# G-Research/ahocorasick_rs

Measured on NVIDIA H100. Metric: haystack_GB_per_s_scanned_find_matches_as_indexes, higher is better.
Workload: dtype u8

## Files before the change

### ahocorasick_rs_b200/csrc/capi.cu

```cuda
#include <atomic>
#include <cstdio>
#include <cstdlib>
#include <cstring>
#include <stdexcept>
#include <string>
#include <utility>
#include <vector>

#include <cooperative_groups.h>

#include "repair.cuh"
#include "scan_staged.cuh"
#include "scan_global.cuh"
#include "scan_sieve.cuh"
#include "tokens.cuh"

namespace acb {

template <int MODE, bool CP>
__global__ void __launch_bounds__(128) scan_plain_kernel(DevImage im, Batch B, Sink out) {
    for (int64_t h = (int64_t)blockIdx.x * blockDim.x + threadIdx.x; h < B.n_haystacks; h += (int64_t)gridDim.x * blockDim.x) {
        const int64_t hs = B.offsets[h], he = B.offsets[h + 1];
        PieceCtx c;
        c.base = B.bytes + hs;
// ... 46 lines not shown
    for (int d = 1; d < 32; d <<= 1) {
        unsigned long long y = __shfl_up_sync(0xffffffffu, x, d);
        if (lane >= d) x += y;
    }
    if (lane == 31) warp_sums[warp] = x;
    __syncthreads();
    if (warp == 0) {
        unsigned long long w = lane < kScanThreads / 32 ? warp_sums[lane] : 0;
#pragma unroll
        for (int d = 1; d < kScanThreads / 32; d <<= 1) {
            unsigned long long y = __shfl_up_sync(0xffffffffu, w, d);
            if (lane >= d) w += y;
        }
        if (lane < kScanThreads / 32) warp_sums[lane] = w;
    }
    __syncthreads();
    const unsigned long long before = warp ? warp_sums[warp - 1] : 0;
    *total = warp_sums[kScanThreads / 32 - 1];
    __syncthreads();
    return before + x - v;
}

template <bool PAIR>
__device__ __forceinline__ unsigned long long scan_item(const uint32_t *in, uint32_t stride, uint64_t i) {
    if (PAIR) {
        const uint2 v = *reinterpret_cast<const uint2 *>(in + i * stride);
        return (unsigned long long)v.x + v.y;
    }
    return in[i * stride];
}

template <bool PAIR>
__device__ __forceinline__ void tile_sum_body(const uint32_t *in, uint32_t stride, uint64_t n, unsigned long long *tile_sums, uint64_t tile,
                                              uint32_t *dense) {
    const uint64_t base = tile * kScanTile + (uint64_t)threadIdx.x * kScanItems;
    unsigned long long v = 0;
#pragma unroll
    for (int i = 0; i < kScanItems; i++)
        if (base + i < n) {
            const unsigned long long x = scan_item<PAIR>(in, stride, base + i);
            if (dense) dense[base + i] = (uint32_t)x;
            v += x;
        }
    unsigned long long total;
    block_exclusive_scan(v, &total);
    if (threadIdx.x == 0) tile_sums[tile] = total;
}

__device__ __forceinline__ unsigned long long tile_prefix(const unsigned long long *tile_sums, uint64_t tile) {
    unsigned long long v = 0;
    for (uint64_t i = threadIdx.x; i < tile; i += kScanThreads) v += tile_sums[i];
    unsigned long long total;
    block_exclusive_scan(v, &total);
    return total;
}

template <bool PAIR>
__device__ __forceinline__ void tile_apply_body(const uint32_t *in, uint32_t stride, uint64_t n, const unsigned long long *tile_sums,
                                                unsigned long long *out, uint64_t tile) {
    const unsigned long long tile_start = tile_prefix(tile_sums, tile);
    const uint64_t base = tile * kScanTile + (uint64_t)threadIdx.x * kScanItems;
    unsigned long long vals[kScanItems], v = 0;
#pragma unroll
    for (int i = 0; i < kScanItems; i++) {
        vals[i] = base + i < n ? scan_item<PAIR>(in, stride, base + i) : 0;
        v += vals[i];
    }
    unsigned long long total;
    unsigned long long run = tile_start + block_exclusive_scan(v, &total);
#pragma unroll
    for (int i = 0; i < kScanItems; i++) {
        if (base + i < n) out[base + i] = run;
        run += vals[i];
        if (base + i + 1 == n) out[n] = run;
    }
}

constexpr int kAccQueue = 0;
constexpr int kAccContFar = 1;
constexpr int kAccRaw = 2;
constexpr int kAccGroups = 3;
constexpr int kAccTraps = 4;
constexpr int kAccRepairs = 5;
constexpr int kAccWords = 8;
constexpr int kAnyScratchWords = 3;

constexpr unsigned kPathFarCp = 1u;
constexpr unsigned kPathSearch = 2u;
constexpr unsigned kPathRepaired = 4u;

struct EpilogueArgs {
    DevImage im;
    Batch B;
    SegPlan P;
    Sink out;
    SegOut seg;
    const uint32_t *counts;
    uint64_t n_items;
    uint8_t *masks;
    unsigned long long *tile_sums, *unit_offsets;
    unsigned long long *cont_tiles, *cont_cum;
    unsigned long long *totals, *acc;
    const acb_match *raw;
    const uint32_t *raw_seq, *raw_unit, *raw_aux;
    unsigned long long raw_cap;
    const uint32_t *pat_cplen;
    acb_match *out_buf;
    unsigned long long out_cap;
    unsigned long long *match_offsets;
    unsigned int *need_repair;
    int do_repair;
};

__device__ __forceinline__ void count_tile(const EpilogueArgs &E, uint64_t tile, bool check, bool with_c0, unsigned int &dirty) {
    const uint64_t n = E.n_items;
    const uint64_t base = tile * kScanTile + (uint64_t)threadIdx.x * kScanItems;
    uint32_t x[kScanItems];
    if (base + kScanItems <= n && !with_c0) {
        const uint4 a = *reinterpret_cast<const uint4 *>(E.counts + base), b = *reinterpret_cast<const uint4 *>(E.counts + base + 4);
        x[0] = a.x, x[1] = a.y, x[2] = a.z, x[3] = a.w, x[4] = b.x, x[5] = b.y, x[6] = b.z, x[7] = b.w;
    } else {
#pragma unroll
        for (int i = 0; i < kScanItems; i++) x[i] = base + i < n ? E.counts[base + i] + (with_c0 ? E.seg.count0[base + i] : 0u) : 0u;
    }
    unsigned long long v = 0;
    uint32_t bits = 0;
#pragma unroll
    for (int i = 0; i < kScanItems; i++) {
        v += x[i];
        bits |= (x[i] != 0u) << i;
    }
    if (check && base < n) {
        uint32_t prev_end = base ? E.seg.key[base - 1].y : kNoState;
#pragma unroll
        for (int i = 0; i < kScanItems; i++)
            if (base + i < n) {
                const uint2 k = E.seg.key[base + i];
                dirty |= (base + i > 0 && k.x != kNoState && k.x != prev_end) ? 1u : 0u;
                prev_end = k.y;
            }
    }
    if (base < n) E.masks[base / kScanItems] = (uint8_t)bits;
    unsigned long long total;
    block_exclusive_scan(v, &total);
    if (threadIdx.x == 0) E.tile_sums[tile] = total;
}

__device__ __forceinline__ void offsets_tile(const EpilogueArgs &E, uint64_t tile, bool with_c0) {
    const uint64_t n = E.n_items;
    const unsigned long long tile_start = tile_prefix(E.tile_sums, tile);
    const uint64_t base = tile * kScanTile + (uint64_t)threadIdx.x * kScanItems;
    const uint32_t bits = base < n ? E.masks[base / kScanItems] : 0u;
    uint32_t x[kScanItems];
    unsigned long long v = 0;
#pragma unroll
    for (int i = 0; i < kScanItems; i++) {
        x[i] = (bits >> i) & 1u ? E.counts[base + i] + (with_c0 ? E.seg.count0[base + i] : 0u) : 0u;
        v += x[i];
    }
    unsigned long long total;
    unsigned long long run = tile_start + block_exclusive_scan(v, &total);
#pragma unroll
    for (int i = 0; i < kScanItems; i++) {
        if ((bits >> i) & 1u) E.unit_offsets[base + i] = run;
        run += x[i];
        if (base + i + 1 == n) E.unit_offsets[n] = run;
    }
}

__device__ __forceinline__ void order_body(const EpilogueArgs &E, unsigned long long raw_total, bool codepoints, bool repaired, bool far) {
    const bool segments = E.seg.key != nullptr;
    const unsigned long long n = raw_total < E.raw_cap ? raw_total : E.raw_cap;
    for (unsigned long long i = (unsigned long long)blockIdx.x * blockDim.x + threadIdx.x; i < n;
         i += (unsigned long long)gridDim.x * blockDim.x) {
        const uint32_t u = E.raw_unit[i];
        uint32_t seq = E.raw_seq[i];
        unsigned long long dst;
        if (segments) {
            const uint32_t k = u >> 1;
            if (repaired && (u & 1u)) {
                const uint32_t drop = E.seg.rest[k].drop;
                if (seq < drop) continue;
                seq += E.seg.count0[k] - drop;
            }
            dst = E.unit_offsets[k] + seq;
        } else {
            dst = E.unit_offsets[u] + seq;
        }
        if (dst >= E.out_cap) continue;
        uint4 r = reinterpret_cast<const uint4 *>(E.raw)[i];
        if (codepoints) {
            unsigned long long cont = E.raw_aux[i];
            if (segments) {
                const int64_t j = u >> 1;
                const int64_t hs = E.B.offsets[r.x];
                if (hs < E.P.origin + j * (int64_t)E.P.seg_bytes) {
                    const int64_t j0 = (hs - E.P.origin) / (int64_t)E.P.seg_bytes;
                    if (far)
                        cont += E.cont_cum[j] - E.cont_cum[j0];
                    else
                        for (int64_t t = j0; t < j; t++) cont += E.seg.cont_tail[t];
                }
            }
            const uint32_t end_cp = r.w - (uint32_t)cont;
            r.w = end_cp;
            r.z = end_cp - E.pat_cplen[r.y];
        }
        reinterpret_cast<uint4 *>(E.out_buf)[dst] = r;
    }
}

__device__ __forceinline__ void match_offsets_body(const EpilogueArgs &E, unsigned long long raw_total, unsigned paths) {
    const unsigned long long total = E.unit_offsets[E.n_items];
    const bool complete = raw_total <= E.raw_cap && total <= E.out_cap;
    const unsigned long long avail = total < E.out_cap ? total : E.out_cap;
    const int64_t nh = E.B.n_haystacks;
    const acb_match *out = E.out_buf;
    const bool run_fill = complete && avail <= 4 * (unsigned long long)(nh + 1);
    if (run_fill) {
        const uint32_t lane = threadIdx.x & 31;
        for (unsigned long long wb = (unsigned long long)blockIdx.x * blockDim.x + (threadIdx.x & ~31u); wb <= avail;
             wb += (unsigned long long)gridDim.x * blockDim.x) {
            const unsigned long long i = wb + lane;
            int64_t hp = 0, hc = 0;
            if (i <= avail) {
                hp = i ? (int64_t)out[i - 1].haystack : -1;
                hc = i < avail ? (int64_t)out[i].haystack : nh;
            }
            unsigned int pending = __ballot_sync(0xffffffffu, hc > hp);
            while (pending) {
                const int src = __ffs(pending) - 1;
                pending &= pending - 1;
                const int64_t a = __shfl_sync(0xffffffffu, hp, src) + 1, b = __shfl_sync(0xffffffffu, hc, src);
                const unsigned long long val = __shfl_sync(0xffffffffu, i, src);
                for (int64_t h = a + lane; h <= b; h += 32) E.match_offsets[h] = val;
            }
        }
    } else {
        for (int64_t h = (int64_t)blockIdx.x * blockDim.x + threadIdx.x; h <= nh; h += (int64_t)gridDim.x * blockDim.x) {
            unsigned long long lo = 0, hi = avail;
            while (lo < hi) {
                const unsigned long long mid = (lo + hi) >> 1;
                if ((int64_t)out[mid].haystack < h)
                    lo = mid + 1;
                else
                    hi = mid;
            }
            E.match_offsets[h] = (h == nh) ? total : lo;
        }
    }
    if (blockIdx.x == 0 && threadIdx.x == 0) {
        unsigned long long *totals = E.totals, *acc = E.acc;
        totals[0] = total;
        totals[1] = complete ? 1 : 0;
        totals[2] = acc[kAccGroups];
        totals[3] = acc[kAccTraps];
        totals[4] = raw_total;
        totals[5] = acc[kAccRepairs];
        totals[6] = paths | (run_fill ? 0u : kPathSearch);
        totals[7] = 0;
        acc[kAccRaw] = acc[kAccGroups] = acc[kAccTraps] = acc[kAccRepairs] = 0;
        acc[kAccQueue] = 0;
        acc[kAccContFar] = 0;
    }
}

template <int MODE, bool CP>
__global__ void __launch_bounds__(kScanThreads) epilogue_kernel(EpilogueArgs E) {
    namespace cg = cooperative_groups;
    cg::grid_group grid = cg::this_grid();
    const bool segments = E.seg.key != nullptr;
    const uint64_t tiles = (E.n_items + kScanTile - 1) / kScanTile;
    unsigned int dirty = 0;
    for (uint64_t tt = blockIdx.x; tt < tiles; tt += gridDim.x) count_tile(E, tt, E.do_repair != 0, false, dirty);
    if (E.do_repair && __any_sync(0xffffffffu, dirty) && (threadIdx.x & 31) == 0) atomicOr(E.need_repair, 1u);
    grid.sync();
    const bool repaired = E.do_repair && *reinterpret_cast<volatile unsigned int *>(E.need_repair);
    if (repaired) {
        for (uint64_t k = (uint64_t)blockIdx.x * blockDim.x + threadIdx.x; k < E.n_items; k += (uint64_t)gridDim.x * blockDim.x)
            E.seg.count0[k] = 0;
        grid.sync();
        repair_body<MODE, CP>(E.im, E.B, E.P, E.out, E.seg, E.acc + kAccRepairs);
        grid.sync();
        for (uint64_t tt = blockIdx.x; tt < tiles; tt += gridDim.x) count_tile(E, tt, false, true, dirty);
        grid.sync();
    }
    const bool far = CP && segments && *reinterpret_cast<volatile unsigned int *>(E.seg.cont_far);
    const uint64_t ctiles = far ? tiles : 0;
    if (far) {
        for (uint64_t tt = blockIdx.x; tt < ctiles; tt += gridDim.x)
            tile_sum_body<false>(E.seg.cont_tail, 1, E.n_items, E.cont_tiles, tt, nullptr);
        grid.sync();
    }
    for (uint64_t tt = blockIdx.x; tt < tiles + ctiles; tt += gridDim.x) {
        if (tt >= tiles)
            tile_apply_body<false>(E.seg.cont_tail, 1, E.n_items, E.cont_tiles, E.cont_cum, tt - tiles);
        else
            offsets_tile(E, tt, repaired);
    }
    grid.sync();
    const unsigned long long raw_total = *reinterpret_cast<volatile unsigned long long *>(E.acc + kAccRaw);
    order_body(E, raw_total, CP, repaired, far);
    grid.sync();
    match_offsets_body(E, raw_total, (far ? kPathFarCp : 0u) | (repaired ? kPathRepaired : 0u));
}


struct SieveEpiArgs {
    Batch B;
    uint32_t *unit_counts;
    uint64_t n_tasks;
    unsigned long long *tile_sums, *unit_offsets;
    const uint32_t *cont_tail;
    const uint32_t *hay_cont;
    unsigned long long *cont_tiles, *cont_cum;
    const acb_match *raw;
    const uint32_t *raw_seq, *raw_unit, *raw_aux;
    unsigned long long raw_cap;
    acb_match *ordered;
    acb_match *final_out;
    unsigned long long out_cap;
    const uint32_t *pat_cplen;
    int64_t origin;
    uint32_t task_bytes;
    uint32_t max_pat_len;
    int longest;
    unsigned long long *totals, *acc, *match_offsets;
};

__device__ __forceinline__ unsigned long long first_of_haystack(const acb_match *list, unsigned long long n, int64_t h) {
    unsigned long long lo = 0, hi = n;
    while (lo < hi) {
        const unsigned long long mid = (lo + hi) >> 1;
        if ((int64_t)list[mid].haystack < h)
            lo = mid + 1;
        else
            hi = mid;
    }
    return lo;
}

template <int MODE, bool PACK = true>
__device__ __forceinline__ uint32_t select_non_overlapping(acb_match *r, unsigned long long n, uint32_t max_len, int longest) {
    unsigned long long w = 0;
    uint32_t s = 0;
    if (MODE == kModeStandard) {
        for (unsigned long long i = 0; i < n; i++) {
            const uint4 m = reinterpret_cast<const uint4 *>(r)[i];
            if (m.z >= s) {
                if (PACK)
                    reinterpret_cast<uint4 *>(r)[w++] = m;
                else
                    w++;
                s = m.w;
            }
        }
        return (uint32_t)w;
    }
    unsigned long long i = 0;
    while (i < n) {
        bool have = false;
        uint4 best = make_uint4(0, 0, 0, 0);
        for (unsigned long long j = i; j < n; j++) {
            const uint4 m = reinterpret_cast<const uint4 *>(r)[j];
            if (have && m.w > best.z + max_len) break;
            if (m.z < s) continue;
            bool better = !have || m.z < best.z;
            if (have && m.z == best.z) better = longest ? (m.w > best.w || (m.w == best.w && m.y < best.y)) : (m.y < best.y);
            if (better) {
                best = m;
                have = true;
            }
        }
        if (!have) break;
        if (PACK)
            reinterpret_cast<uint4 *>(r)[w++] = best;
        else
            w++;
        s = best.w;
        while (i < n && r[i].end <= s) i++;
    }
    return (uint32_t)w;
}

template <bool CP>
__device__ __forceinline__ void sieve_order_list(const SieveEpiArgs &E, cooperative_groups::grid_group &grid) {
    const uint64_t tiles = (E.n_tasks + kScanTile - 1) / kScanTile;
// ... 1679 lines not shown
    const int64_t cap = (int64_t)d.sms * 16;
    if (blocks > cap) blocks = cap;
    if (blocks < 1) blocks = 1;
    scan_plain_kernel<MODE, CP><<<(unsigned)blocks, threads, 0, st>>>(im, B, out);
    g_launches++;
    return ACB_OK;
}

template <int MODE, bool CP, int COLMODE, int V>
int launch_staged(const DevImage &im, const DevHot &hot, const Batch &B, const SegPlan &P, const Sink &out, const SegOut &seg_out,
                  const DeviceInfo &d, unsigned int *task_counter, unsigned long long *trap_stats, cudaStream_t st) {
    auto kern = scan_staged_kernel<MODE, CP, COLMODE, V>;
    constexpr int kWarpsMax = V == 1 ? kMaxWarps : kMaxWarps2;
    const uint64_t q = P.lane_stride;
    const uint64_t tasks = ((uint64_t)P.n_segments + 32 * V * q - 1) / (32 * V * q) * q;
    const int ctas = d.sms;
    int warps = (int)((tasks + ctas - 1) / ctas);
    if (warps < 4) warps = 4;
    if (warps > kWarpsMax) warps = kWarpsMax;
    const uint32_t row_bytes = COLMODE == kColAscii ? kAsciiCols * 2 : im.n_cols * 2;
    const uint32_t stage_bytes = (uint32_t)warps * V * (2 * kStageBytes + kMetaBytes);
    const uint32_t budget = (uint32_t)d.max_smem_optin;
    if (budget < stage_bytes + kStageOffset + 3 * (row_bytes + 4) + 256) return fail(ACB_ECUDA, "not enough shared memory for the staged kernel");
    uint32_t rows = (budget - stage_bytes - kStageOffset - 256) / (row_bytes + 4);
    if (rows > (60u * 1024u) / row_bytes) rows = (60u * 1024u) / row_bytes;
    if (COLMODE == kColAscii) rows -= 1;
    uint32_t H = rows - 1;
    const uint32_t have = COLMODE == kColAscii ? hot.n_rows128 : hot.n_rows;
    if (H > have) H = have;
    if (g_tuning.hot_rows > 0 && (uint32_t)g_tuning.hot_rows < H) H = (uint32_t)g_tuning.hot_rows;
    if (H < 1) return fail(ACB_ECUDA, "rows too wide for the staged kernel");
    const uint32_t hot_bytes = (((H + 1 + (COLMODE == kColAscii ? 1 : 0)) * row_bytes) + 127u) & ~127u;
    const uint32_t smem = hot_bytes + kStageOffset + (((H + 1) * 4 + 127u) & ~127u) + stage_bytes;
    CUDA_OK(cudaFuncSetAttribute(kern, cudaFuncAttributeMaxDynamicSharedMemorySize, (int)budget));
    kern<<<ctas, warps * 32, smem, st>>>(im, hot, B, P, out, seg_out, H, hot_bytes, task_counter, trap_stats);
    g_launches++;
    return ACB_OK;
}

uint32_t ascii_rows_that_fit(const DeviceInfo &d) {
    const uint32_t stage_bytes = (uint32_t)kMaxWarps * (2 * kStageBytes + kMetaBytes);
    const uint32_t budget = (uint32_t)d.max_smem_optin;
    if (budget < stage_bytes + kStageOffset + 128 + 2 * kAsciiCols * 2) return 0;
    uint32_t rows = (budget - stage_bytes - kStageOffset - 256) / (kAsciiCols * 2 + 4);
    if (rows > (60u * 1024u) / (kAsciiCols * 2)) rows = (60u * 1024u) / (kAsciiCols * 2);
    return rows - 2;
}

template <int MODE, bool CP>
int launch_staged_cols(const ImageHeader &h, const DevImage &im, const DevHot &hot, const Batch &B, const SegPlan &P, const Sink &out,
                       const SegOut &seg_out, const DeviceInfo &d, unsigned int *task_counter, unsigned long long *trap_stats,
                       cudaStream_t st, bool ascii, int per_lane) {
#define ACB_GO(COLS)                                                                                                        \
    (per_lane == 2 ? launch_staged<MODE, CP, COLS, 2>(im, hot, B, P, out, seg_out, d, task_counter, trap_stats, st)      \
                   : launch_staged<MODE, CP, COLS, 1>(im, hot, B, P, out, seg_out, d, task_counter, trap_stats, st))
    if (ascii) return ACB_GO(kColAscii);
    if (h.col_mode == kColRange) return ACB_GO(kColRange);
    return ACB_GO(kColClass);
#undef ACB_GO
}

template <int MODE, bool CP>
int launch_global(const DevImage &im, const Batch &B, const SegPlan &P, const Sink &out, const SegOut &seg_out, const DeviceInfo &d,
                  cudaStream_t st) {
    int64_t blocks = (P.n_segments + 255) / 256;
    const int64_t cap = (int64_t)d.sms * 64;
    if (blocks > cap) blocks = cap;
    if (blocks < 1) blocks = 1;
    scan_global_kernel<MODE, CP><<<(unsigned)blocks, 256, 0, st>>>(im, B, P, out, seg_out);
    g_launches++;
    return ACB_OK;
}

inline int epilogue_blocks_per_sm(int max_bps, uint64_t n_units) {
    static const int forced = [] {
        const char *e = std::getenv("ACB200_EPILOGUE_BPS");
        return e ? std::atoi(e) : 0;
    }();
    (void)n_units;
    int b = forced > 0 ? forced : max_bps;
    return b > max_bps ? max_bps : (b < 1 ? 1 : b);
}

template <int MODE, bool CP>
int launch_epilogue(EpilogueArgs &E, const DeviceInfo &d, cudaStream_t st) {
    auto kern = epilogue_kernel<MODE, CP>;
    static thread_local int blocks_per_sm[3][2] = {{0, 0}, {0, 0}, {0, 0}};
    static thread_local int cached_device = -1;
    if (cached_device != d.device) {
        for (auto &row : blocks_per_sm) row[0] = row[1] = 0;
        cached_device = d.device;
    }
    int &bps = blocks_per_sm[MODE][CP ? 1 : 0];
    if (bps == 0) {
        CUDA_OK(cudaOccupancyMaxActiveBlocksPerMultiprocessor(&bps, kern, kScanThreads, 0));
        if (bps < 1) return fail(ACB_ECUDA, "epilogue kernel does not fit on an SM");
        if (bps > 4) bps = 4;
    }
    void *args[] = {&E};
    const int use_bps = epilogue_blocks_per_sm(bps, E.n_items);
    CUDA_OK(cudaLaunchCooperativeKernel(reinterpret_cast<void *>(kern), dim3(d.sms * use_bps), dim3(kScanThreads), args, 0, st));
    g_launches++;
    return ACB_OK;
}


DevSieve make_sieve_view(const SieveHeader &h, const void *dev_sieve) {
    const uint8_t *b = static_cast<const uint8_t *>(dev_sieve);
    DevSieve v;
    v.bloom = reinterpret_cast<const uint32_t *>(b + h.off_bloom);
    v.ht = reinterpret_cast<const SieveSlot *>(b + h.off_ht);
    v.na = reinterpret_cast<const SieveNodeA *>(b + h.off_node_a);
    v.nb = reinterpret_cast<const SieveNodeB *>(b + h.off_node_b);
    v.pids = reinterpret_cast<const uint32_t *>(b + h.off_pids);
    v.W = h.W;
    v.last_level = h.last_level;
    v.n_probes = h.n_probes;
    v.bloom_words = h.bloom_words;
    v.prim_words = h.prim_words;
    v.ht_size = h.ht_mask + 1;
    v.max_pat_len = h.max_pat_len;
    v.term_levels = h.term_levels;
    return v;
}

template <bool CP, int MODE = kSieveList>
int launch_sieve(const DevSieve &sv, const Batch &B, SievePlan &P, const Sink &out, uint32_t *task_cont, uint32_t *hay_cont,
                 unsigned int *task_counter, const DeviceInfo &d, cudaStream_t st, const SieveFilter *F = nullptr) {
    const uint32_t ring = acb_sieve_ring(sv.bloom_words * 4, (uint32_t)d.max_smem_optin);
    if (ring == 0) return fail(ACB_ECUDA, "the sieve's filters do not fit in shared memory (rebuild them with a smaller bloom_bytes_max)");
    const uint32_t smem = sieve_smem_bytes(sv.bloom_words * 4, ring, CP);
    P.ring = ring;
#define ACB_SIEVE_GO(WC)                                                                                      \
    do {                                                                                                      \
        if constexpr (MODE != kSievePatterns) {                                                               \
            if (F) {                                                                                          \
                auto kern = sieve_scan_filtered_kernel<CP, WC, MODE>;                                         \
                CUDA_OK(cudaFuncSetAttribute(kern, cudaFuncAttributeMaxDynamicSharedMemorySize, d.max_smem_optin)); \
                kern<<<d.sms, kSieveThreads, smem, st>>>(sv, B, P, out, task_cont, hay_cont, task_counter, *F); \
                break;                                                                                        \
            }                                                                                                 \
        }                                                                                                     \
        auto kern = sieve_scan_kernel<CP, WC, MODE>;                                                          \
        CUDA_OK(cudaFuncSetAttribute(kern, cudaFuncAttributeMaxDynamicSharedMemorySize, d.max_smem_optin));   \
        kern<<<d.sms, kSieveThreads, smem, st>>>(sv, B, P, out, task_cont, hay_cont, task_counter);           \
    } while (0)
    if (sv.W < 4)
        ACB_SIEVE_GO(0);
    else if (sv.W == 4)
        ACB_SIEVE_GO(1);
    else if (sv.W == 5)
        ACB_SIEVE_GO(3);
    else
        ACB_SIEVE_GO(2);
#undef ACB_SIEVE_GO
    g_launches++;
    return ACB_OK;
}

template <int MODE, bool CP>
int launch_sieve_epilogue(SieveEpiArgs &E, const DeviceInfo &d, cudaStream_t st) {
    auto kern = sieve_epilogue_kernel<MODE, CP>;
    static thread_local int blocks_per_sm[3][2] = {{0, 0}, {0, 0}, {0, 0}};
    static thread_local int cached_device = -1;
    if (cached_device != d.device) {
        for (auto &row : blocks_per_sm) row[0] = row[1] = 0;
        cached_device = d.device;
    }
    int &bps = blocks_per_sm[MODE][CP ? 1 : 0];
    if (bps == 0) {
        CUDA_OK(cudaOccupancyMaxActiveBlocksPerMultiprocessor(&bps, kern, kScanThreads, 0));
        if (bps < 1) return fail(ACB_ECUDA, "epilogue kernel does not fit on an SM");
        if (bps > 4) bps = 4;
    }
    void *args[] = {&E};
    const uint64_t n_work = E.n_tasks > (uint64_t)E.B.n_haystacks ? E.n_tasks : (uint64_t)E.B.n_haystacks;
    const int use_bps = epilogue_blocks_per_sm(bps, n_work);
    CUDA_OK(cudaLaunchCooperativeKernel(reinterpret_cast<void *>(kern), dim3(d.sms * use_bps), dim3(kScanThreads), args, 0, st));
    g_launches++;
    return ACB_OK;
// ... 679 lines not shown
    (mode == kModeStandard   ? (cp ? FN<kModeStandard, true>(__VA_ARGS__) : FN<kModeStandard, false>(__VA_ARGS__)) \
     : mode == kModeLeftmost ? (cp ? FN<kModeLeftmost, true>(__VA_ARGS__) : FN<kModeLeftmost, false>(__VA_ARGS__)) \
                             : (cp ? FN<kModeOverlap, true>(__VA_ARGS__) : FN<kModeOverlap, false>(__VA_ARGS__)))
    if (segments) {
        P.origin = -(int64_t)(reinterpret_cast<uintptr_t>(dev_bytes) & 63u);
        P.seg_bytes = plan->segment_bytes;
        P.warm = plan->warm_bytes;
        P.n_segments = (int64_t)plan->n_segments;
        P.lane_stride = plan->lane_stride;
        P.avg_len = n_haystacks > 0 ? total_bytes / (uint64_t)n_haystacks : 0;
    }
    SegOut seg_out{};
    if (segments) {
        uint8_t *si = static_cast<uint8_t *>(ws->dev_seg_info);
        const uint64_t n = plan->n_segments;
        seg_out.rest = reinterpret_cast<SegRest *>(si);
        seg_out.key = reinterpret_cast<uint2 *>(si + 16 * n);
        seg_out.cont_tail = cp ? reinterpret_cast<uint32_t *>(si + 24 * n) : nullptr;
        seg_out.count = ws->dev_unit_counts;
        seg_out.count0 = ws->dev_unit_counts + n;
        seg_out.cont_far = reinterpret_cast<unsigned int *>(acc + kAccContFar);
    }
    if (kernel == 4) {
        rc = ACB_DISPATCH(launch_global, im, B, P, out, seg_out, d, st);
        if (rc) return rc;
        CUDA_OK(cudaGetLastError());
        if (ev1) {
            CUDA_OK(cudaEventRecord(ev1, st));
            g_timing_events.emplace_back(ev0, ev1);
        }
    } else if (segments) {
        DevHot hot;
        if ((rc = make_hot_view(a, dev_hot, *hot_desc, hot))) return rc;
        uint32_t fit128 = ascii_rows_that_fit(d);
        if (fit128 > hot.n_rows128) fit128 = hot.n_rows128;
        if (g_tuning.hot_rows > 0 && (uint32_t)g_tuning.hot_rows < fit128) fit128 = (uint32_t)g_tuning.hot_rows;
        const bool ascii = g_tuning.table == 2 && fit128 > 0 && per_lane == 1;
        rc = ACB_DISPATCH(launch_staged_cols, h, im, hot, B, P, out, seg_out, d, task_counter, acc + kAccGroups, st, ascii, per_lane);
        if (rc) return rc;
        CUDA_OK(cudaGetLastError());
        if (ev1) {
            CUDA_OK(cudaEventRecord(ev1, st));
            g_timing_events.emplace_back(ev0, ev1);
        }
    } else {
        rc = ACB_DISPATCH(launch_plain, im, B, out, d, st);
        if (rc) return rc;
        CUDA_OK(cudaGetLastError());
        if (ev1) {
            CUDA_OK(cudaEventRecord(ev1, st));
            g_timing_events.emplace_back(ev0, ev1);
        }
    }
    const uint64_t max_tiles = (plan->n_units + kScanTile - 1) / kScanTile;
    unsigned long long *tile_sums = acc + kAccWords;
    unsigned long long *cont_tiles = tile_sums + max_tiles + 1;
    unsigned long long *cont_cum = cont_tiles + max_tiles + 1;
    EpilogueArgs E;
    E.im = im;
    E.B = B;
    E.P = P;
    E.out = out;
    E.seg = seg_out;
    E.counts = ws->dev_unit_counts;
    E.n_items = segments ? plan->n_segments : (uint64_t)n_haystacks;
    E.masks = reinterpret_cast<uint8_t *>(acc + want.scratch_words - (plan->n_units / 64 + 2));
    E.tile_sums = tile_sums;
    E.unit_offsets = unit_offsets;
    E.cont_tiles = cont_tiles;
    E.cont_cum = cont_cum;
    E.totals = totals;
    E.acc = acc;
    E.raw = ws->dev_raw;
    E.raw_seq = ws->dev_raw_seq;
    E.raw_unit = ws->dev_raw_unit;
    E.raw_aux = ws->dev_raw_aux;
    E.raw_cap = ws->raw_capacity;
    E.pat_cplen = im.pat_cplen;
    E.out_buf = ws->dev_out;
    E.out_cap = ws->out_capacity;
    E.match_offsets = match_offsets;
    E.need_repair = task_counter + 1;
    E.do_repair = (segments && mode != kModeOverlap) ? 1 : 0;
    rc = ACB_DISPATCH(launch_epilogue, E, d, st);
#undef ACB_DISPATCH
    if (rc) return rc;
    CUDA_OK(cudaGetLastError());
    return ACB_OK;
}

int acb_scan_batch(const acb_automaton *a, const void *dev_image, const void *dev_hot, const acb_hot_desc *hot_desc,
                   const void *dev_sieve, const uint8_t *dev_bytes, const int64_t *dev_offsets, int64_t n_haystacks, uint64_t total_bytes,
                   int overlapping, int codepoints, const acb_plan *plan, const acb_workspace *ws, void *stream) {
    return acb_scan_batch_filtered(a, dev_image, dev_hot, hot_desc, dev_sieve, dev_bytes, dev_offsets, n_haystacks, total_bytes, overlapping,
                                   codepoints, plan, ws, nullptr, stream);
}

int acb_stream_seams(const acb_automaton *a, const uint8_t *dev_bytes, const int64_t *dev_offsets, int64_t n_streams, uint64_t total_bytes,
                     const int64_t *dev_carry, const uint8_t *dev_tail, uint8_t *dev_seam_bytes, int64_t *dev_seam_offsets, void *stream) {
    if (!a || !dev_offsets || !dev_carry || !dev_seam_offsets || (total_bytes && !dev_bytes)) return fail(ACB_EINVAL, "null argument");
    const uint32_t halo = a->impl->hdr.max_pat_len ? a->impl->hdr.max_pat_len - 1 : 0;
    if (halo && (!dev_tail || !dev_seam_bytes)) return fail(ACB_EINVAL, "null argument");
    if (n_streams < 0 || n_streams > 0xfffffffell) return fail(ACB_EINVAL, "n_streams out of range (0 .. 2^32 - 2)");
    if (total_bytes >= (1ull << 31)) return fail(ACB_EINVAL, "total_bytes must be below 2^31 (feed larger data in more chunks)");
    DeviceInfo d;
    if (int rc = device_info(d)) return rc;
    cudaStream_t st = static_cast<cudaStream_t>(stream);
    if (n_streams == 0) {
        CUDA_OK(cudaMemsetAsync(dev_seam_offsets, 0, sizeof(int64_t), st));
        return ACB_OK;
    }
    int64_t blocks = (n_streams + 255) / 256;
    if (blocks > 8ll * d.sms) blocks = 8ll * d.sms;
    stream_seam_lengths_kernel<<<(unsigned)blocks, 256, 0, st>>>(dev_offsets, n_streams, dev_carry, halo, dev_seam_offsets);
    stream_prefix_kernel<<<1, kScanThreads, 0, st>>>(dev_seam_offsets, n_streams);
    int64_t fill_blocks = (n_streams + 7) / 8;
    if (fill_blocks > 16ll * d.sms) fill_blocks = 16ll * d.sms;
    if (halo)
        stream_seam_fill_kernel<<<(unsigned)fill_blocks, 256, 0, st>>>(dev_bytes, dev_offsets, n_streams, dev_carry, dev_tail, halo,
                                                                       dev_seam_offsets, dev_seam_bytes);
    g_launches += halo ? 3 : 2;
    CUDA_OK(cudaGetLastError());
    return ACB_OK;
}

int acb_stream_resolve(const acb_automaton *a, const void *dev_image, const uint8_t *dev_bytes, const int64_t *dev_offsets, int64_t n_streams,
                       uint64_t total_bytes, const uint8_t *dev_last, int overlapping, int codepoints, int64_t *dev_carry, uint8_t *dev_tail,
                       const uint8_t *dev_seam_bytes, const int64_t *dev_seam_offsets, const acb_match *dev_seam_list,
                       const uint64_t *dev_seam_match_offsets, const acb_match *dev_chunk_list, const uint64_t *dev_chunk_match_offsets,
                       int64_t *dev_scratch, int64_t *dev_rows, int64_t *dev_row_offsets, void *stream) {
    if (!a || !dev_offsets || !dev_carry || !dev_seam_offsets || !dev_seam_list || !dev_seam_match_offsets || !dev_chunk_list ||
        !dev_chunk_match_offsets || !dev_scratch || !dev_rows || !dev_row_offsets || (total_bytes && !dev_bytes))
        return fail(ACB_EINVAL, "null argument");
    const ImageHeader &h = a->impl->hdr;
    const int kind = (int)h.match_kind;
    if (overlapping != 0 && overlapping != 1) return fail(ACB_EINVAL, "overlapping must be 0 or 1");
    if (overlapping && kind != ACB_STANDARD)
        return fail(ACB_EUNSUPPORTED, std::string("match kind ") + (kind == ACB_LEFTMOST_FIRST ? "LeftmostFirst" : "LeftmostLongest") +
                                          " does not support overlapping searches");
    const uint32_t halo = h.max_pat_len ? h.max_pat_len - 1 : 0;
    if (halo && (!dev_tail || !dev_seam_bytes)) return fail(ACB_EINVAL, "null argument");
    if (codepoints && !dev_image) return fail(ACB_EINVAL, "code points need the device image (pattern lengths in code points)");
    if (n_streams < 0 || n_streams > 0xfffffffell) return fail(ACB_EINVAL, "n_streams out of range (0 .. 2^32 - 2)");
    if (total_bytes >= (1ull << 31)) return fail(ACB_EINVAL, "total_bytes must be below 2^31 (feed larger data in more chunks)");
    DeviceInfo d;
    if (int rc = device_info(d)) return rc;
    cudaStream_t st = static_cast<cudaStream_t>(stream);
    CUDA_OK(cudaMemsetAsync(dev_scratch, 0, 2 * sizeof(uint64_t), st));
    if (n_streams == 0) {
        CUDA_OK(cudaMemsetAsync(dev_row_offsets, 0, sizeof(int64_t), st));
        return ACB_OK;
    }
    StreamArgs A;
    A.B = Batch{dev_bytes, dev_offsets, n_streams};
    A.carry = dev_carry;
    A.tail = dev_tail;
    A.last = dev_last;
    A.seam = dev_seam_bytes;
    A.seam_offsets = dev_seam_offsets;
    A.seam_list = reinterpret_cast<const uint4 *>(dev_seam_list);
    A.chunk_list = reinterpret_cast<const uint4 *>(dev_chunk_list);
    A.seam_mo = reinterpret_cast<const unsigned long long *>(dev_seam_match_offsets);
    A.chunk_mo = reinterpret_cast<const unsigned long long *>(dev_chunk_match_offsets);
    A.stats = reinterpret_cast<unsigned long long *>(dev_scratch);
    A.cont_rows = reinterpret_cast<long long *>(dev_scratch + 2);
    A.cont_cp = reinterpret_cast<long long *>(dev_scratch + 2 + 3 * n_streams);
// ... 212 lines not shown
```

### ahocorasick_rs_b200/matcher.py

```python
from __future__ import annotations

import ctypes as C
import enum
import threading
from typing import Iterable, Optional, Sequence

import numpy as np

from . import _capi


class MatchKind(enum.Enum):
    Standard = 0
    LeftmostFirst = 1
    LeftmostLongest = 2


class Implementation(enum.Enum):
    NoncontiguousNFA = 0
    ContiguousNFA = 1
    DFA = 2


_TRACE = bool(__import__("os").environ.get("ACB200_TRACE"))
# ... 1128 lines not shown
                self.mask_device(hay[w0:w1], torch.tensor([0, w1 - w0], dtype=torch.int64, device=dev), True, flt=flt, words=words,
                                 bit_base=bit_base + w0)
                if w1 == hay.numel():
                    return
                w0 += limit - halo
        rows = self._scan_one_large(hay, False, False, flt)
        self._mask_rows(words, bit_base, rows, torch.tensor([0, hay.numel()], dtype=torch.int64, device=dev))

    def unpack_mask(self, words, n: int, stride: int = 1):
        torch = _require_cuda()
        out = torch.empty(n, dtype=torch.bool, device=words.device)
        rc = self._L.acb_mask_unpack(words.data_ptr(), 0, stride, n, out.data_ptr(), torch.cuda.current_stream(words.device).cuda_stream)
        if rc != _capi.ACB_OK:
            raise RuntimeError(_capi.last_error())
        return out

    def spans_host_batch(self, chunks: Sequence[bytes], overlapping, codepoints: bool, patterns=None, unit: int = 1):
        torch = _require_cuda()
        self.check_overlapping(overlapping)
        n = len(chunks)
        if n == 0:
            return []
        offs = np.zeros(n + 1, dtype=np.int64)
        np.cumsum(np.fromiter((len(c) for c in chunks), dtype=np.int64, count=n), out=offs[1:])
        total_bytes = int(offs[-1])
        head = (8 * (n + 1) + 511) & ~511
        dev = torch.device("cuda", torch.cuda.current_device())
        with self._host_lock:
            host = self._pinned(head + total_bytes)
            hv = host.numpy()
            hv[:8 * (n + 1)].view(np.int64)[:] = offs
            if n == 1:
                hv[head:head + total_bytes] = np.frombuffer(chunks[0], dtype=np.uint8)
            elif total_bytes:
                hv[head:head + total_bytes] = np.frombuffer(b"".join(chunks), dtype=np.uint8)
            d = host[:head + total_bytes].to(dev, non_blocking=True)
            flt = _host_sets(self, patterns, n, dev) if patterns is not None else None
            words = self.mask_device(d[head:], d[:8 * (n + 1)].view(torch.int64), overlapping, flt=flt).cpu().numpy()
            text = hv[head:head + total_bytes].copy() if codepoints else None
        return spans_from_words(words, offs, text, unit)

    def scan_device(self, data, offsets, overlapping=False, codepoints=False, capacity: Optional[int] = None,
                    sync: bool = True, ws_slot: int = 0, flt=None):
        torch = _require_cuda()
        self.check_overlapping(overlapping)
        dev = data.device
        n = offsets.numel() - 1
        if data.numel() > self.WINDOW_BYTES:
            if not sync:
                raise ValueError(f"buffers above {self.WINDOW_BYTES} bytes are scanned in windows: sync=False is not available")
            return self._scan_device_windows(data, offsets, overlapping, codepoints, flt)
        img = self.image(dev)
        cap = capacity or max(1024, n * 2)
        stream = torch.cuda.current_stream(dev).cuda_stream
        with self._lock, torch.cuda.device(dev):
            hot = self._pick_engine(dev, data, offsets, overlapping) if flt is None else None
            use_sieve = hot is None
            if use_sieve:
                sieve_t, sieve_d = self.sieve(dev)
            plan = self._plan(data, n)
            while True:
                ws = self._workspace(dev, plan, n, cap, ws_slot)
                reader = ws.pop("reader", None)
                if reader is not None:
                    torch.cuda.current_stream(dev).wait_event(reader)
                st = self._ws_struct(ws)
                rc = self._L.acb_scan_batch_filtered(self._h, img.data_ptr(),
                                                     hot["tensor"].data_ptr() if hot else None, C.byref(hot["rows"]) if hot else None,
                                                     sieve_t.data_ptr() if use_sieve else None,
                                                     data.data_ptr(), offsets.data_ptr(), n, data.numel(),
                                                     2 if overlapping == 2 else int(bool(overlapping)), int(bool(codepoints)), C.byref(plan),
                                                     C.byref(st), _filter_struct(flt), stream)
                if rc != _capi.ACB_OK:
                    err = _capi.last_error()
                    ws["scratch"][:8].zero_()
                    raise (ValueError if rc == _capi.ACB_EUNSUPPORTED else RuntimeError)(err)
                if not sync:
                    return ws["out"], ws["match_offsets"][: n + 1], ws["total"]
                tot = ws["total"].tolist()
                total, complete, raw_total = tot[0], tot[1], tot[4]
                if hot:
                    self._note_trap_stats(hot, tot[2], tot[3])
                    self.last_stats = {"engine": "table", "groups": tot[2], "traps": tot[3], "repairs": tot[5], "segments": plan.n_segments,
                                       "paths": tot[6],
                                       "hot_rows": hot["rows"].rows, "hot_rows128": hot["rows"].rows128,
                                       "hot_visited": hot["rows"].visited, "hot_coverage": round(hot.get("coverage", 1.0), 5),
                                       "global_table": bool(hot["rows"].reserved & 1),
                                       "segment_bytes": plan.segment_bytes, "lane_stride": plan.lane_stride}
                else:
                    self.last_stats = {"engine": "sieve", **self.sieve_geometry(dev, plan.task_bytes), "nodes": sieve_d.nodes,
                                       "keys": sieve_d.keys, "filter_entries": sieve_d.filter_entries, "list_records": raw_total,
                                       **self._set_stats(flt)}
                if complete or (total == 0 and raw_total == 0):
                    return ws["out"][:total], ws["match_offsets"][: n + 1], total
                cap = max(total, raw_total) + max(total, raw_total) // 8 + 16

    WINDOW_BYTES = (1 << 31) - (1 << 16)

    def _scan_device_windows(self, data, offsets, overlapping, codepoints, flt=None):
        torch = _require_cuda()
        dev = data.device
        n = offsets.numel() - 1
        limit = self.WINDOW_BYTES
        parts = []
        mo = torch.zeros(n + 1, dtype=torch.int64, device=dev)
        lens = offsets[1:] - offsets[:-1]
        oversized = bool((lens > limit).any().item()) if n else False
        base_count = 0
        h = 0
        while h < n:
            start = int(offsets[h].item())
            if oversized and int(lens[h].item()) > limit:
                part = self._scan_one_large(data[start:start + int(lens[h].item())], overlapping, codepoints, _filter_slice(flt, h, h + 1))
                part[:, 0] = h
                parts.append(part)
                base_count += int(part.shape[0])
                mo[h + 1] = base_count
                h += 1
                continue
            h1 = int(torch.searchsorted(offsets, torch.tensor([start + limit], dtype=torch.int64, device=dev), right=True).item()) - 1
            h1 = max(h + 1, min(h1, n))
            if oversized:
                big = torch.nonzero(lens[h:h1] > limit)
                if big.numel():
                    h1 = h + int(big[0].item())
            end = int(offsets[h1].item())
            sub_offs = offsets[h:h1 + 1] - start
            _t0 = __import__("time").perf_counter() if _TRACE else 0
            m, mo_run, total = self.scan_device(data[start:end], sub_offs, overlapping, codepoints, flt=_filter_slice(flt, h, h1))
            _t1 = __import__("time").perf_counter() if _TRACE else 0
            part = m.to(torch.int64)
            if h:
                part[:, 0] += h
            parts.append(part)
            mo[h + 1:h1 + 1] = mo_run[1:h1 - h + 1].to(torch.int64) + base_count
            base_count += int(total)
            if _TRACE:
                torch.cuda.synchronize()
                print(f"[trace] run haystacks {h}..{h1} ({end - start} B): scan_device {(_t1 - _t0) * 1e3:.2f} ms, post {(__import__('time').perf_counter() - _t1) * 1e3:.2f} ms, total {total}", flush=True)
            h = h1
        out = torch.cat(parts, dim=0) if len(parts) != 1 else parts[0]
        if not parts:
            out = torch.zeros((0, 4), dtype=torch.int64, device=dev)
        return out, mo, int(out.shape[0])

    def _scan_one_large(self, hay, overlapping, codepoints, flt=None):
        torch = _require_cuda()
        dev = hay.device
        rows = self._overlapping_rows_large(hay, codepoints, flt)
        if overlapping or rows.shape[0] == 0:
            return rows
        rows = rows.contiguous()
        out = torch.empty_like(rows)
        count = torch.zeros(1, dtype=torch.int64, device=dev)
        rc = self._L.acb_select_non_overlapping(self._h, rows.data_ptr(), rows.shape[0], out.data_ptr(), count.data_ptr(),
                                                torch.cuda.current_stream(dev).cuda_stream)
        if rc != _capi.ACB_OK:
            raise RuntimeError(_capi.last_error())
        return out[: int(count.item())]

    def _overlapping_rows_large(self, hay, codepoints, flt=None):
        torch = _require_cuda()
        dev = hay.device

        def scan_window(window):
            one = torch.tensor([0, window.numel()], dtype=torch.int64, device=dev)
            m, _, _ = self._scan_overlapping_list(window, one, codepoints, flt)
# ... 1381 lines not shown
```

Before: 1658.

## Add single-pass fast epilogue kernel with decoupled tile lookback for sparse matches

Adds an epilogue_fast_kernel that, when the match count is small, does the count scan, the record ordering and the match-offset computation in one pass. It uses per-tile status words with a random tag for decoupled lookback, so no cooperative grid syncs are needed. On success it sets a tag that makes the following cooperative epilogue kernel exit at once. This targets the launch and grid-sync latency of the multi-phase epilogue in low-match workloads. In exchange it adds an extra launch, spin-waits on tile status (which relies on earlier tiles being resident), and falls back to the slow path if it gives up.

Result: no change. 1690, median of 6 (+1.9%).

```diff
diff --git a/ahocorasick_rs_b200/csrc/capi.cu b/ahocorasick_rs_b200/csrc/capi.cu
--- a/ahocorasick_rs_b200/csrc/capi.cu
+++ b/ahocorasick_rs_b200/csrc/capi.cu
@@ -152,6 +152,8 @@
 constexpr int kAccGroups = 3;
 constexpr int kAccTraps = 4;
 constexpr int kAccRepairs = 5;
+constexpr int kAccFastDone = 6;
+constexpr int kAccFastTag = 7;
 constexpr int kAccWords = 8;
 constexpr int kAnyScratchWords = 3;
 
@@ -180,6 +182,8 @@
     unsigned long long *match_offsets;
     unsigned int *need_repair;
     int do_repair;
+    unsigned long long *tile_status;
+    unsigned long long fast_tag;
 };
 
 __device__ __forceinline__ void count_tile(const EpilogueArgs &E, uint64_t tile, bool check, bool with_c0, unsigned int &dirty) {
@@ -236,6 +240,28 @@
         run += x[i];
         if (base + i + 1 == n) E.unit_offsets[n] = run;
     }
+}
+
+__device__ __forceinline__ uint4 load_record(const EpilogueArgs &E, unsigned long long i, uint32_t u, bool codepoints, bool far) {
+    uint4 r = reinterpret_cast<const uint4 *>(E.raw)[i];
+    if (codepoints) {
+        unsigned long long cont = E.raw_aux[i];
+        if (E.seg.key != nullptr) {
+            const int64_t j = u >> 1;
+            const int64_t hs = E.B.offsets[r.x];
+            if (hs < E.P.origin + j * (int64_t)E.P.seg_bytes) {
+                const int64_t j0 = (hs - E.P.origin) / (int64_t)E.P.seg_bytes;
+                if (far)
+                    cont += E.cont_cum[j] - E.cont_cum[j0];
+                else
+                    for (int64_t t = j0; t < j; t++) cont += E.seg.cont_tail[t];
+            }
+        }
+        const uint32_t end_cp = r.w - (uint32_t)cont;
+        r.w = end_cp;
+        r.z = end_cp - E.pat_cplen[r.y];
+    }
+    return r;
 }
 
 __device__ __forceinline__ void order_body(const EpilogueArgs &E, unsigned long long raw_total, bool codepoints, bool repaired, bool far) {
@@ -257,27 +283,24 @@
         } else {
             dst = E.unit_offsets[u] + seq;
         }
-        if (dst >= E.out_cap) continue;
-        uint4 r = reinterpret_cast<const uint4 *>(E.raw)[i];
-        if (codepoints) {
-            unsigned long long cont = E.raw_aux[i];
-            if (segments) {
-                const int64_t j = u >> 1;
-                const int64_t hs = E.B.offsets[r.x];
-                if (hs < E.P.origin + j * (int64_t)E.P.seg_bytes) {
-                    const int64_t j0 = (hs - E.P.origin) / (int64_t)E.P.seg_bytes;
-                    if (far)
-                        cont += E.cont_cum[j] - E.cont_cum[j0];
-                    else
-                        for (int64_t t = j0; t < j; t++) cont += E.seg.cont_tail[t];
-                }
-            }
-            const uint32_t end_cp = r.w - (uint32_t)cont;
-            r.w = end_cp;
-            r.z = end_cp - E.pat_cplen[r.y];
-        }
-        reinterpret_cast<uint4 *>(E.out_buf)[dst] = r;
-    }
+        if (dst < E.out_cap) reinterpret_cast<uint4 *>(E.out_buf)[dst] = load_record(E, i, u, codepoints, far);
+    }
+}
+
+__device__ __forceinline__ void publish_totals(const EpilogueArgs &E, unsigned long long total, bool complete, unsigned long long raw_total,
+                                               unsigned paths, bool fast) {
+    unsigned long long *totals = E.totals, *acc = E.acc;
+    totals[0] = total;
+    totals[1] = complete ? 1 : 0;
+    totals[2] = acc[kAccGroups];
+    totals[3] = acc[kAccTraps];
+    totals[4] = raw_total;
+    totals[5] = acc[kAccRepairs];
+    totals[6] = paths;
+    totals[7] = fast ? 1 : 0;
+    acc[kAccRaw] = acc[kAccGroups] = acc[kAccTraps] = acc[kAccRepairs] = 0;
+    acc[kAccQueue] = 0;
+    acc[kAccContFar] = 0;
 }
 
 __device__ __forceinline__ void match_offsets_body(const EpilogueArgs &E, unsigned long long raw_total, unsigned paths) {
@@ -319,25 +342,24 @@
             E.match_offsets[h] = (h == nh) ? total : lo;
         }
     }
-    if (blockIdx.x == 0 && threadIdx.x == 0) {
-        unsigned long long *totals = E.totals, *acc = E.acc;
-        totals[0] = total;
-        totals[1] = complete ? 1 : 0;
-        totals[2] = acc[kAccGroups];
-        totals[3] = acc[kAccTraps];
-        totals[4] = raw_total;
-        totals[5] = acc[kAccRepairs];
-        totals[6] = paths | (run_fill ? 0u : kPathSearch);
-        totals[7] = 0;
-        acc[kAccRaw] = acc[kAccGroups] = acc[kAccTraps] = acc[kAccRepairs] = 0;
-        acc[kAccQueue] = 0;
-        acc[kAccContFar] = 0;
-    }
-}
+    if (blockIdx.x == 0 && threadIdx.x == 0) publish_totals(E, total, complete, raw_total, paths | (run_fill ? 0u : kPathSearch), false);
+}
+
+#ifdef ACB_EPILOGUE_STOP_AFTER
+#define ACB_EPILOGUE_STOP(N)                                                                                         \
+    if (ACB_EPILOGUE_STOP_AFTER == (N)) {                                                                            \
+        if (blockIdx.x == 0 && threadIdx.x == 0) publish_totals(E, 0, false, 0, 0, false);                          \
+        return;                                                                                                      \
+    }
+#else
+#define ACB_EPILOGUE_STOP(N)
+#endif
 
 template <int MODE, bool CP>
 __global__ void __launch_bounds__(kScanThreads) epilogue_kernel(EpilogueArgs E) {
     namespace cg = cooperative_groups;
+    if (E.fast_tag && *reinterpret_cast<volatile unsigned long long *>(E.acc + kAccFastTag) == E.fast_tag) return;
+    ACB_EPILOGUE_STOP(0)
     cg::grid_group grid = cg::this_grid();
     const bool segments = E.seg.key != nullptr;
     const uint64_t tiles = (E.n_items + kScanTile - 1) / kScanTile;
@@ -345,6 +367,7 @@
     for (uint64_t tt = blockIdx.x; tt < tiles; tt += gridDim.x) count_tile(E, tt, E.do_repair != 0, false, dirty);
     if (E.do_repair && __any_sync(0xffffffffu, dirty) && (threadIdx.x & 31) == 0) atomicOr(E.need_repair, 1u);
     grid.sync();
+    ACB_EPILOGUE_STOP(1)
     const bool repaired = E.do_repair && *reinterpret_cast<volatile unsigned int *>(E.need_repair);
     if (repaired) {
         for (uint64_t k = (uint64_t)blockIdx.x * blockDim.x + threadIdx.x; k < E.n_items; k += (uint64_t)gridDim.x * blockDim.x)
@@ -369,10 +392,173 @@
             offsets_tile(E, tt, repaired);
     }
     grid.sync();
+    ACB_EPILOGUE_STOP(2)
     const unsigned long long raw_total = *reinterpret_cast<volatile unsigned long long *>(E.acc + kAccRaw);
     order_body(E, raw_total, CP, repaired, far);
     grid.sync();
+    ACB_EPILOGUE_STOP(3)
     match_offsets_body(E, raw_total, (far ? kPathFarCp : 0u) | (repaired ? kPathRepaired : 0u));
+}
+
+constexpr unsigned long long kFastRecords = 4 * kScanTile;
+constexpr unsigned kFastTileRecords = kScanTile;
+constexpr int kRawPerThread = kFastRecords / kScanThreads;
+constexpr unsigned long long kTileSumMask = 0xfff;
+
+template <bool CP>
+__global__ void __launch_bounds__(kScanThreads) epilogue_fast_kernel(EpilogueArgs E) {
+    const uint64_t n = E.n_items, tile = blockIdx.x;
+    const int64_t nh = E.B.n_haystacks;
+    const unsigned long long raw_total = *reinterpret_cast<volatile unsigned long long *>(E.acc + kAccRaw);
+    if ((CP && *reinterpret_cast<volatile unsigned int *>(E.seg.cont_far)) || raw_total > E.raw_cap || raw_total > E.out_cap ||
+        raw_total > 4 * (unsigned long long)(nh + 1) || raw_total > kFastRecords)
+        return;
+    volatile unsigned long long *status = E.tile_status;
+    __shared__ uint32_t s_local[kScanTile];
+    __shared__ uint4 s_rec[kFastTileRecords];
+    __shared__ uint16_t s_list[kFastTileRecords];
+    __shared__ unsigned int s_found;
+    if (threadIdx.x == 0) s_found = 0;
+    uint32_t u[kRawPerThread];
+#pragma unroll
+    for (int j = 0; j < kRawPerThread; j++) {
+        const unsigned long long i = (unsigned long long)j * kScanThreads + threadIdx.x;
+        u[j] = i < raw_total ? __ldg(E.raw_unit + i) : 0xffffffffu;
+    }
+
+    const int half = threadIdx.x >> 7, t = threadIdx.x & 127;
+    const int64_t pos0 = E.P.origin + (int64_t)(tile * kScanTile) * (int64_t)E.P.seg_bytes;
+    const int64_t pos1 = pos0 + (int64_t)kScanTile * (int64_t)E.P.seg_bytes;
+    int64_t lo0 = 0, hi0 = tile > 0 ? nh + 1 : 0;
+    int64_t lo1 = (tile + 1) * kScanTile < n ? 0 : nh + 1, hi1 = nh + 1;
+    auto guess = [&](int64_t pos) {
+        const int64_t g = E.P.avg_len && pos > 0 ? pos / (int64_t)E.P.avg_len - 64 : 0, top = nh + 1 - 128;
+        return g < top ? (g > 0 ? g : 0) : (top > 0 ? top : 0);
+    };
+    const int64_t g0 = guess(pos0), g1 = guess(pos1), p = (half ? g1 : g0) + t;
+    const bool below = p <= nh && E.B.offsets[p] < (half ? pos1 : pos0);
+
+    const uint64_t base = tile * kScanTile + (uint64_t)threadIdx.x * kScanItems;
+    uint32_t x[kScanItems];
+    unsigned long long v = 0;
+    unsigned int dirty = 0;
+    uint32_t prev_end = base && base < n ? E.seg.key[base - 1].y : kNoState;
+#pragma unroll
+    for (int i = 0; i < kScanItems; i++) {
+        x[i] = base + i < n ? E.counts[base + i] : 0u;
+        v += x[i];
+        if (E.do_repair && base + i < n) {
+            const uint2 k = E.seg.key[base + i];
+            dirty |= (base + i > 0 && k.x != kNoState && k.x != prev_end) ? 1u : 0u;
+            prev_end = k.y;
+        }
+    }
+    unsigned long long agg;
+    const unsigned long long excl = block_exclusive_scan(v, &agg);
+    const uint64_t k_lo = tile * kScanTile;
+#pragma unroll
+    for (int j = 0; j < kRawPerThread; j++) {
+        const uint64_t k = u[j] >> 1;
+        if (u[j] != 0xffffffffu && k >= k_lo && k < k_lo + kScanTile) {
+            const unsigned int slot = atomicAdd(&s_found, 1u);
+            if (slot < kFastTileRecords) s_list[slot] = (uint16_t)(j * kScanThreads + threadIdx.x);
+        }
+    }
+    const unsigned long long tag = E.fast_tag & ~kTileSumMask;
+    const bool gave_up = __syncthreads_or(dirty) != 0 || agg > kFastTileRecords || s_found != agg;
+    if (threadIdx.x == 0) status[tile] = tag | (gave_up ? 0ull : agg);
+    {
+        uint32_t run = (uint32_t)excl;
+#pragma unroll
+        for (int i = 0; i < kScanItems; i++) {
+            s_local[threadIdx.x * kScanItems + i] = run;
+            run += x[i];
+        }
+    }
+
+    {
+        const int c0 = __syncthreads_count(half == 0 && below), c1 = __syncthreads_count(half == 1 && below);
+        auto settle = [&](int64_t &lo, int64_t &hi, int64_t g, int c) {
+            const int64_t w = nh + 1 - g < 128 ? nh + 1 - g : 128;
+            if (lo >= hi) return;
+            if (c == 0)
+                hi = g < hi ? g : hi;
+            else if (c == w)
+                lo = g + w > lo ? g + w : lo;
+            else
+                lo = hi = g + c;
+        };
+        settle(lo0, hi0, g0, c0);
+        settle(lo1, hi1, g1, c1);
+    }
+    while (lo0 < hi0 || lo1 < hi1) {
+        const int64_t step0 = (hi0 - lo0 + 127) / 128, step1 = (hi1 - lo1 + 127) / 128;
+        const int64_t lo = half ? lo1 : lo0, hi = half ? hi1 : hi0, step = half ? step1 : step0;
+        const int64_t q = lo + (int64_t)(t + 1) * step - 1;
+        const bool b = lo < hi && q < hi && E.B.offsets[q] < (half ? pos1 : pos0);
+        const int c0 = __syncthreads_count(half == 0 && b), c1 = __syncthreads_count(half == 1 && b);
+        const int64_t nhi0 = lo0 + (int64_t)(c0 + 1) * step0 - 1, nhi1 = lo1 + (int64_t)(c1 + 1) * step1 - 1;
+        lo0 += (int64_t)c0 * step0;
+        hi0 = nhi0 < hi0 ? nhi0 : hi0;
+        lo1 += (int64_t)c1 * step1;
+        hi1 = nhi1 < hi1 ? nhi1 : hi1;
+    }
+
+    if (!gave_up) {
+        for (unsigned int q = threadIdx.x; q < agg; q += kScanThreads) {
+            const uint32_t i = s_list[q], unit = E.raw_unit[i];
+            const uint32_t local = s_local[(unit >> 1) - k_lo] + E.raw_seq[i];
+            if (local < kFastTileRecords) s_rec[local] = load_record(E, i, unit, CP, false);
+        }
+    }
+
+    unsigned long long w = 0;
+    for (uint64_t j = threadIdx.x; j < tile; j += kScanThreads) {
+        unsigned long long s;
+        while (((s = status[j]) & ~kTileSumMask) != tag) {
+        }
+        w += s & kTileSumMask;
+    }
+    unsigned long long start;
+    block_exclusive_scan(w, &start);
+    if (!gave_up) {
+        unsigned long long run = start + excl;
+#pragma unroll
+        for (int i = 0; i < kScanItems; i++) {
+            if (x[i]) E.unit_offsets[base + i] = run;
+            run += x[i];
+            if (base + i + 1 == n) E.unit_offsets[n] = run;
+        }
+        for (uint32_t j = threadIdx.x; j < agg; j += kScanThreads)
+            if (start + j < E.out_cap) reinterpret_cast<uint4 *>(E.out_buf)[start + j] = s_rec[j];
+        for (int64_t h = lo0 + threadIdx.x; h < lo1; h += kScanThreads) {
+            uint32_t a = 0, b = (uint32_t)agg;
+            while (a < b) {
+                const uint32_t mid = (a + b) >> 1;
+                if ((int64_t)s_rec[mid].x < h)
+                    a = mid + 1;
+                else
+                    b = mid;
+            }
+            E.match_offsets[h] = start + a;
+        }
+    }
+
+    __syncthreads();
+    if (threadIdx.x == 0) {
+        __threadfence();
+        const unsigned long long before = atomicAdd(E.acc + kAccFastDone, 1ull | ((unsigned long long)gave_up << 32));
+        if ((uint32_t)before == gridDim.x - 1) {
+            __threadfence();
+            const unsigned long long total = *reinterpret_cast<volatile unsigned long long *>(E.unit_offsets + n);
+            const bool done = (before >> 32) == 0 && !gave_up && total <= E.out_cap && total <= 4 * (unsigned long long)(nh + 1);
+            if (done) {
+                publish_totals(E, total, true, raw_total, 0u, true);
+                E.acc[kAccFastTag] = E.fast_tag;
+            }
+            E.acc[kAccFastDone] = 0;
+        }
+    }
 }
 
 
@@ -2218,6 +2404,15 @@
     return b > max_bps ? max_bps : (b < 1 ? 1 : b);
 }
 
+unsigned long long next_step_tag() {
+    static std::atomic<unsigned long long> counter{0};
+    unsigned long long z = ++counter * 0x9e3779b97f4a7c15ull;
+    z = (z ^ (z >> 30)) * 0xbf58476d1ce4e5b9ull;
+    z = (z ^ (z >> 27)) * 0x94d049bb133111ebull;
+    z ^= z >> 31;
+    return z >> 12 ? z : 1ull << 12;
+}
+
 template <int MODE, bool CP>
 int launch_epilogue(EpilogueArgs &E, const DeviceInfo &d, cudaStream_t st) {
     auto kern = epilogue_kernel<MODE, CP>;
@@ -2232,6 +2427,13 @@
         CUDA_OK(cudaOccupancyMaxActiveBlocksPerMultiprocessor(&bps, kern, kScanThreads, 0));
         if (bps < 1) return fail(ACB_ECUDA, "epilogue kernel does not fit on an SM");
         if (bps > 4) bps = 4;
+    }
+    E.fast_tag = 0;
+    const char *fast = std::getenv("ACB200_EPILOGUE_FAST");
+    if (E.seg.key && E.tile_status && !(fast && std::strcmp(fast, "0") == 0)) {
+        E.fast_tag = next_step_tag();
+        epilogue_fast_kernel<CP><<<(unsigned)((E.n_items + kScanTile - 1) / kScanTile), kScanThreads, 0, st>>>(E);
+        g_launches++;
     }
     void *args[] = {&E};
     const int use_bps = epilogue_blocks_per_sm(bps, E.n_items);
@@ -3077,6 +3279,7 @@
     E.match_offsets = match_offsets;
     E.need_repair = task_counter + 1;
     E.do_repair = (segments && mode != kModeOverlap) ? 1 : 0;
+    E.tile_status = segments ? cont_cum : nullptr;
     rc = ACB_DISPATCH(launch_epilogue, E, d, st);
 #undef ACB_DISPATCH
     if (rc) return rc;
diff --git a/ahocorasick_rs_b200/matcher.py b/ahocorasick_rs_b200/matcher.py
--- a/ahocorasick_rs_b200/matcher.py
+++ b/ahocorasick_rs_b200/matcher.py
@@ -1234,7 +1234,7 @@
                 if hot:
                     self._note_trap_stats(hot, tot[2], tot[3])
                     self.last_stats = {"engine": "table", "groups": tot[2], "traps": tot[3], "repairs": tot[5], "segments": plan.n_segments,
-                                       "paths": tot[6],
+                                       "paths": tot[6], "epilogue_fast": tot[7],
                                        "hot_rows": hot["rows"].rows, "hot_rows128": hot["rows"].rows128,
                                        "hot_visited": hot["rows"].visited, "hot_coverage": round(hot.get("coverage", 1.0), 5),
                                        "global_table": bool(hot["rows"].reserved & 1),
```
